# stdio2016/pfann

Measured on AMD Instinct MI355X. Metric: query segments/sec, 10 s @ SNR 0 queries vs 1M-segment db (exact flat IP top-100 + sequence match), higher is better.
Workload: dtype f32

## Files before the change

include/pfann_amd.h:

```cpp
#ifndef PFANN_AMD_H
#define PFANN_AMD_H

#include <stdint.h>

#ifdef __cplusplus
extern "C" {
#endif

#define PFANN_SEQSCORE_VERSION 20220625002LL


long long version(void);

int seq_score(void *index, const int64_t *song_pos, int n_songs, const float *query,
              int query_len, const int64_t *labels, int top_k, float *song_scores,
              int frame_shift_mul, float score_alpha);

const char *pfann_last_error(void);

typedef struct pfann_ctx pfann_ctx;

typedef struct pfann_config {
    int32_t segment_len;
    int32_t stft_n;
// ... 4 lines not shown
    int32_t log_mode;
    int32_t spec_norm_max;
    float   log_eps;
    int32_t d, h, u;
    int32_t fuller;
    int32_t activation;
    int32_t relu_after_bn;
    int32_t stride_t[8];
    int32_t stride_f[8];
    int32_t max_batch;
} pfann_config;

pfann_ctx *pfann_create(const pfann_config *cfg, int device);
void pfann_destroy(pfann_ctx *ctx);

int pfann_set_melbank(pfann_ctx *ctx, const float *fb_host, int n_freqs, int n_mels);

int pfann_load_weight(pfann_ctx *ctx, const char *name, const float *host, int64_t numel);
int pfann_weights_missing(pfann_ctx *ctx);

int pfann_melspec(pfann_ctx *ctx, const float *segs_dev, int64_t B, int64_t seg_stride,
                  int remove_mean, float *out_dev, void *stream);

int pfann_melspec_plan(pfann_ctx *ctx, int64_t B, int out[4]);

int pfann_encode(pfann_ctx *ctx, const float *mel_dev, int64_t B, float *emb_dev,
                 int normalize, void *stream);

int pfann_segment_embed(pfann_ctx *ctx, const float *wav_dev, int64_t B, int64_t seg_stride,
                        float *emb_dev, int normalize, void *stream);

int pfann_segment_embed_at(pfann_ctx *ctx, const float *wav_dev, const int64_t *starts_dev,
                           int64_t B, float *emb_dev, int normalize, void *stream);

int pfann_pcm16_to_mono(pfann_ctx *ctx, const int16_t *pcm_dev, int64_t n_frames, int n_ch,
                        float *wav_dev, void *stream);

int pfann_pcm16_files_to_mono(pfann_ctx *ctx, const void *const *host_pcm, const int64_t *n_samples, const int64_t *dst_off,
                              int n_files, int16_t *pcm_dev, int64_t total, float *wav_dev, void *stream);

typedef struct pfann_wav_info {
    int64_t n_frames;
    int64_t data_pos;
    int32_t n_ch;
    int32_t sample_rate;
    int32_t status;
    int32_t reserved;
// ... 213 lines not shown
```

pfann_amd/csrc/api.hip:

```cpp
#include <math.h>
#include <stdarg.h>
#include <stdlib.h>
#include <string.h>

#include <algorithm>
#include <cmath>
#include <map>
#include <mutex>

#include "kernels.h"
#include "search_plan.h"

namespace pfann { int launch_rows_to_half(const float *x, int64_t n, int d, void *xh, float *norm_max_dev, hipStream_t s); }

__global__ void noop_api_kernel() {}
static int launch_noop_api() {
    hipLaunchKernelGGL(noop_api_kernel, dim3(1), dim3(1), 0, 0);
    return hipGetLastError() == hipSuccess ? 0 : -1;
}

namespace pfann {

static thread_local char g_err[1024] = "";
void set_error(const char *fmt, ...) {
// ... 61 lines not shown
    int keep = 0;
    int64_t keep_first = 0;
    int64_t keep_B = 0;
    float *dbg[16] = {};
    bool dbg_has[16] = {};
    float *dbg_tmp = nullptr;
    int64_t dbg_cap = 0;
};

extern "C" int pfann_set_streams(pfann_ctx *c, int n);

static int build_plan(pfann_ctx *c) {
    const char *why = plan_sublayers(c->cfg, c->F, c->T, c->sub);
    if (why) { set_error("%s", why); return -1; }
    return 0;
}

static int upload(float **dst, const float *src, size_t n) {
    if (*dst == nullptr) PF_HIP(hipMalloc(dst, n * sizeof(float)));
    PF_HIP(hipMemcpy(*dst, src, n * sizeof(float), hipMemcpyHostToDevice));
    return 0;
}

__global__ void pfann_bench_region_marker() {}

extern "C" {

long long version(void) { return PFANN_SEQSCORE_VERSION; }

const char *pfann_last_error(void) { return g_err; }

pfann_ctx *pfann_create(const pfann_config *cfg, int device) {
    if (hipSetDevice(device) != hipSuccess) { set_error("hipSetDevice(%d) failed: no usable GPU", device); return nullptr; }
    pfann_ctx *c = new pfann_ctx();
    c->cfg = *cfg;
    c->device = device;
    if (c->cfg.max_batch <= 0) c->cfg.max_batch = 512;
    const int n_fft = cfg->stft_n;
    int log2n = 0;
    while ((1 << log2n) < n_fft) ++log2n;
    if ((1 << log2n) != n_fft || n_fft < 64 || n_fft > 4096) { set_error("stft_n must be a power of two in 64..4096"); delete c; return nullptr; }
    if (cfg->n_mels % 1 != 0 || cfg->n_mels <= 0) { set_error("bad n_mels"); delete c; return nullptr; }
    MelPlan &m = c->mel;
    memset(&m, 0, sizeof(m));
    m.seg_len = cfg->segment_len; m.n_fft = n_fft; m.hop = cfg->stft_hop; m.n_mels = cfg->n_mels;
    m.n_frames = 1 + cfg->segment_len / cfg->stft_hop;
    m.n_freqs = n_fft / 2 + 1; m.log2n = log2n;
    m.power = cfg->power; m.pad_reflect = cfg->pad_reflect; m.log_mode = cfg->log_mode;
    m.spec_norm_max = cfg->spec_norm_max; m.log_eps = cfg->log_eps;
    if (m.pad_reflect && n_fft / 2 >= cfg->segment_len) { set_error("reflect padding needs stft_n/2 < segment_len"); delete c; return nullptr; }
    std::vector<float> win(n_fft);
    std::vector<float2> tw(n_fft / 2);
    for (int n = 0; n < n_fft; ++n) win[n] = (float)(0.5 - 0.5 * cos(2.0 * M_PI * n / n_fft));
    for (int j = 0; j < n_fft / 2; ++j) {
        tw[j].x = (float)cos(-2.0 * M_PI * j / n_fft);
        tw[j].y = (float)sin(-2.0 * M_PI * j / n_fft);
    }
    if (hipMalloc(&m.window, n_fft * sizeof(float)) != hipSuccess ||
        hipMalloc(&m.twiddle, (n_fft / 2) * sizeof(float2)) != hipSuccess) { set_error("hipMalloc failed"); delete c; return nullptr; }
    (void)hipMemcpy(m.window, win.data(), n_fft * sizeof(float), hipMemcpyHostToDevice);
    (void)hipMemcpy(m.twiddle, tw.data(), (n_fft / 2) * sizeof(float2), hipMemcpyHostToDevice);
    c->F = cfg->n_mels;
    c->T = m.n_frames;
    if (build_plan(c)) { delete c; return nullptr; }
    c->n_expected = 8 * 8 + 4;
    for (int i = 0; i < 16; ++i) {
        const int64_t e = (int64_t)c->sub[i].co * c->sub[i].Fo * c->sub[i].To;
        c->buf_elems[i & 1] = std::max(c->buf_elems[i & 1], e);
    }
    c->fused = fused_supported(c->sub, 16) && getenv("PFANN_NO_FUSE") == nullptr;
    if (!c->fused && cfg->fuller && getenv("PFANN_NO_FUSE") == nullptr)
        fprintf(stderr, "pfann_amd: this model's layer shapes (an Fo*To that is not a power of two, or channel counts not "
// ... 17 lines not shown
        if (c->sub[i].w_hi) { (void)hipFree(c->sub[i].w_hi); (void)hipFree(c->sub[i].w_lo); }
        if (c->sub[i].w22) (void)hipFree(c->sub[i].w22);
        if (c->sub[i].bias) (void)hipFree(c->sub[i].bias);
        if (c->sub[i].ln_w) (void)hipFree(c->sub[i].ln_w);
        if (c->sub[i].ln_b) (void)hipFree(c->sub[i].ln_b);
        if (c->dbg[i]) (void)hipFree(c->dbg[i]);
    }
    float *ptrs[] = {c->g_w1, c->g_b1, c->g_w2, c->g_b2, c->buf[0], c->buf[1], c->part[0], c->part[1], c->splitk, c->stats, c->mel_buf, c->mel.window,
                     c->mel.fb_val, c->dbg_tmp};
    for (float *p : ptrs) if (p) (void)hipFree(p);
    if (c->mel.twiddle) (void)hipFree(c->mel.twiddle);
    if (c->mel.fb_ptr) (void)hipFree(c->mel.fb_ptr);
    if (c->mel.fb_idx) (void)hipFree(c->mel.fb_idx);
    if (c->scratch) (void)hipFree(c->scratch);
    delete c;
}

int pfann_set_melbank(pfann_ctx *c, const float *fb, int n_freqs, int n_mels) {
    if (n_freqs != c->mel.n_freqs || n_mels != c->mel.n_mels) {
        set_error("melbank shape [%d,%d] != [%d,%d]", n_freqs, n_mels, c->mel.n_freqs, c->mel.n_mels);
        return -3;
    }
    PF_HIP(hipSetDevice(c->device));
    std::vector<int> ptr(n_mels + 1, 0), idx;
    std::vector<float> val;
    int mx = 0;
    for (int m = 0; m < n_mels; ++m) {
        for (int k = 0; k < n_freqs; ++k) {
            const float v = fb[(size_t)k * n_mels + m];
            if (v != 0.0f) { idx.push_back(k); val.push_back(v); }
        }
        ptr[m + 1] = (int)idx.size();
        mx = std::max(mx, ptr[m + 1] - ptr[m]);
    }
    if (idx.empty()) { idx.push_back(0); val.push_back(0.f); }
    MelPlan &mp = c->mel;
    if (mp.fb_ptr) { (void)hipFree(mp.fb_ptr); (void)hipFree(mp.fb_idx); (void)hipFree(mp.fb_val); }
    PF_HIP(hipMalloc(&mp.fb_ptr, ptr.size() * sizeof(int)));
    PF_HIP(hipMalloc(&mp.fb_idx, idx.size() * sizeof(int)));
    PF_HIP(hipMalloc(&mp.fb_val, val.size() * sizeof(float)));
    PF_HIP(hipMemcpy(mp.fb_ptr, ptr.data(), ptr.size() * sizeof(int), hipMemcpyHostToDevice));
    PF_HIP(hipMemcpy(mp.fb_idx, idx.data(), idx.size() * sizeof(int), hipMemcpyHostToDevice));
    PF_HIP(hipMemcpy(mp.fb_val, val.data(), val.size() * sizeof(float), hipMemcpyHostToDevice));
    mp.max_nnz_row = mx;
    mp.fb_nnz = (int)idx.size();
    c->mel_ready = true;
    return 0;
}

int pfann_load_weight(pfann_ctx *c, const char *name, const float *host, int64_t numel) {
    PF_HIP(hipSetDevice(c->device));
    const pfann_config &g = c->cfg;
    int blk = -1;
    char mod[16] = "", kind[16] = "";
    if (sscanf(name, "f.convs.%d.%15[a-z0-9].%15s", &blk, mod, kind) == 3 && blk >= 0 && blk < 8) {
        const bool second = mod[strlen(mod) - 1] == '2';
        SubLayer &L = c->sub[2 * blk + (second ? 1 : 0)];
        const bool is_w = strcmp(kind, "weight") == 0;
        if (!is_w && strcmp(kind, "bias") != 0) { set_error("unknown tensor %s", name); return -2; }
        if (strncmp(mod, "conv", 4) == 0) {
            if (!is_w) {
                if (numel != L.co) { set_error("%s: numel %lld != %d", name, (long long)numel, L.co); return -3; }
                if (upload(&L.bias, host, numel)) return -1;
                if (blk == 0 && !second) { c->b1_host.assign(host, host + numel); c->gram_ready = false; }
            } else {
                const int ci = L.depthwise ? 1 : L.ci;
                if (numel != (int64_t)L.co * ci * 3) { set_error("%s: numel %lld != %lld", name, (long long)numel, (long long)L.co * ci * 3); return -3; }
                std::vector<float> w((size_t)numel);
// ... 56 lines not shown
        else if (!strcmp(name, "g.linear1.bias")) { dst = &c->g_b1; want = (int64_t)g.d * g.u; }
        else if (!strcmp(name, "g.linear2.weight")) { dst = &c->g_w2; want = (int64_t)g.d * g.u; }
        else if (!strcmp(name, "g.linear2.bias")) { dst = &c->g_b2; want = g.d; }
        else { set_error("unknown tensor %s", name); return -2; }
        if (numel != want) { set_error("%s: numel %lld != %lld", name, (long long)numel, (long long)want); return -3; }
        if (upload(dst, host, numel)) return -1;
    } else {
        set_error("unknown tensor %s", name);
        return -2;
    }
    c->loaded[name] = true;
    return 0;
}

int pfann_weights_missing(pfann_ctx *c) { return c->n_expected - (int)c->loaded.size(); }

int pfann_melspec(pfann_ctx *c, const float *segs, int64_t B, int64_t seg_stride, int remove_mean, float *out,
                  void *stream) {
    PF_HIP(hipSetDevice(c->device));
    if (!c->mel_ready) { set_error("pfann_melspec: mel filterbank not set"); return -5; }
    return launch_melspec(c->mel, segs, B, seg_stride, nullptr, remove_mean, out, (hipStream_t)stream);
}

int pfann_melspec_plan(pfann_ctx *c, int64_t B, int out[4]) {
    if (!c->mel_ready) { set_error("pfann_melspec_plan: mel filterbank not set"); return -5; }
    const MelLaunch ml = plan_melspec(c->mel, B);
    out[0] = ml.group_out; out[1] = ml.parts; out[2] = (int)ml.lds_bytes; out[3] = ml.radix8;
    return 0;
}

static int64_t keep_window(const pfann_ctx *c, int64_t B, int64_t *first) {
    const int64_t nb = std::min<int64_t>(B, 8);
    *first = std::max<int64_t>(0, std::min<int64_t>(c->keep_first, B - nb));
    return nb;
}

static int keep_tap(pfann_ctx *c, int idx, const float *act, int64_t B, hipStream_t s) {
    const SubLayer &L = c->sub[idx];
    const int64_t e = (int64_t)L.co * L.Fo * L.To;
    int64_t b0;
    const int64_t nb = keep_window(c, B, &b0);
    if (!c->dbg[idx]) PF_HIP(hipMalloc(&c->dbg[idx], 8 * e * sizeof(float)));
    PF_HIP(hipMemcpyAsync(c->dbg[idx], act + b0 * e, nb * e * sizeof(float), hipMemcpyDeviceToDevice, s));
    c->keep_B = nb;
    c->dbg_has[idx] = true;
    return 0;
}

static int ensure_workspace(pfann_ctx *c, bool need_mel) {
    const int64_t mb = c->cfg.max_batch;
// ... 1385 lines not shown
```

pfann_amd/csrc/kernels.h:

```cpp
#pragma once
#include "common.h"
#include "encoder_plan.h"

namespace pfann {

struct MelPlan {
    int seg_len, n_fft, hop, n_mels, n_frames, n_freqs, log2n;
    int power, pad_reflect, log_mode, spec_norm_max;
    float log_eps;
    float *window;
    float2 *twiddle;
    int *fb_ptr;
    int *fb_idx;
    float *fb_val;
    int max_nnz_row, fb_nnz;
};
struct MelLaunch {
    int group_out, parts, radix8;
    size_t lds_bytes;
};
MelLaunch plan_melspec(const MelPlan &mp, int64_t B);
int launch_melspec(const MelPlan &mp, const float *segs, int64_t B, int64_t seg_stride,
                   const int64_t *starts, int remove_mean, float *out, hipStream_t s);
int launch_resample_to_mono(const int16_t *pcm, int n_ch, const float *K, int old_r, int new_r, int width, const int64_t *plan,
                            int n_pieces, int64_t n_out, float *tmp, float *wav, float *scratch2, hipStream_t s);
int launch_pcm16_to_mono(const int16_t *pcm, int64_t n_frames, int n_ch, float *wav,
                         float *scratch2, hipStream_t s);

int launch_conv_first(const SubLayer &L, const float *x, float *y, int64_t B, hipStream_t s);
int launch_conv_gemm(const SubLayer &L, const float *x, float *y, int64_t B, hipStream_t s, int64_t Bcall = 0);
int launch_conv_depthwise(const SubLayer &L, const float *x, float *y, int64_t B, hipStream_t s);
int launch_ln_act(const SubLayer &L, float *xy, int64_t B, int activation, int relu_after_bn,
                  hipStream_t s);
int launch_myg(const float *x, const float *w1, const float *b1, const float *w2, const float *b2,
               int d, int u, int v, int64_t B, float *emb, int normalize, hipStream_t s);
int launch_cl_to_nchw(const float *x, float *y, int64_t B, int C, int HW, hipStream_t s);

bool fused_supported(const SubLayer *sub, int n);
int fused_out_slots(const SubLayer &L, int64_t B);
int launch_conv_first_stats(const SubLayer &L, const float *x, float *y, float *part, int64_t B, int act,
                            int after_bn, hipStream_t s);
int launch_conv_first_gram_stats(const SubLayer &L, const float *x, float *part, int64_t B, const float *gram14,
                                 hipStream_t s);
// ... 195 lines not shown
```

pfann_amd/csrc/mel.hip:

```cpp
#include <stdlib.h>

#include "kernels.h"

namespace pfann {

struct MelArgs {
    const float *segs; float *out;
    int64_t seg_stride;
    const int64_t *starts;
    int seg_len, n_fft, hop, n_mels, n_frames, log2n;
    int power, pad_reflect, log_mode, spec_norm_max, remove_mean;
    float log_eps;
    const float *window; const float2 *twiddle;
    const int *fb_ptr, *fb_idx; const float *fb_val;
    int fb_nnz;
    int parts;
    int group_out;
};

__device__ __forceinline__ unsigned bitrev(unsigned x, int bits) { return __brev(x) >> (32 - bits); }

__device__ __forceinline__ float2 cadd(float2 a, float2 b) { return make_float2(a.x + b.x, a.y + b.y); }
__device__ __forceinline__ float2 csub(float2 a, float2 b) { return make_float2(a.x - b.x, a.y - b.y); }
__device__ __forceinline__ float2 cmul(float2 a, float2 b) { return make_float2(a.x * b.x - a.y * b.y, a.x * b.y + a.y * b.x); }
__device__ __forceinline__ float2 mul_mi(float2 a) { return make_float2(a.y, -a.x); }

__device__ __forceinline__ void dft8(float2 (&a)[8]) {
    const float c = 0.70710678118654752440f;
    float2 u[8], v[8];
#pragma unroll
    for (int j = 0; j < 4; ++j) { u[j] = cadd(a[j], a[j + 4]); u[j + 4] = csub(a[j], a[j + 4]); }
    u[5] = make_float2(c * (u[5].x + u[5].y), c * (u[5].y - u[5].x));
    u[6] = mul_mi(u[6]);
    u[7] = make_float2(c * (u[7].y - u[7].x), -c * (u[7].x + u[7].y));
#pragma unroll
    for (int h = 0; h < 8; h += 4) {
        v[h] = cadd(u[h], u[h + 2]); v[h + 2] = csub(u[h], u[h + 2]);
        v[h + 1] = cadd(u[h + 1], u[h + 3]); v[h + 3] = mul_mi(csub(u[h + 1], u[h + 3]));
    }
    a[0] = cadd(v[0], v[1]); a[4] = csub(v[0], v[1]);
    a[2] = cadd(v[2], v[3]); a[6] = csub(v[2], v[3]);
    a[1] = cadd(v[4], v[5]); a[5] = csub(v[4], v[5]);
    a[3] = cadd(v[6], v[7]); a[7] = csub(v[6], v[7]);
}

__global__ __launch_bounds__(256) void melspec_kernel(MelArgs a) {
    extern __shared__ __attribute__((aligned(16))) float smem[];
    const int M = a.n_fft >> 1;
    const int log2m = a.log2n - 1;
    const int n_freqs = M + 1;
    float *tw_re = smem;
    float *tw_im = tw_re + M;
    const int WSZ = 2 * M > 1152 ? 2 * M : 1152;
    float *work = tw_im + M;
    float *pw = work + 4 * WSZ;
    float *tile = pw + 4 * (M + 4);
    const int tp = a.group_out ? a.group_out + 1 : a.n_frames + 1;
    float *red = tile + a.n_mels * tp;
    int *s_ptr = reinterpret_cast<int *>(red + 8);
    int *s_idx = s_ptr + a.n_mels + 1;
    float *s_val = reinterpret_cast<float *>(s_idx + a.fb_nnz);

    const int tid = threadIdx.x, lane = tid & 63, wave = tid >> 6;
    const int seg = a.parts > 1 ? (int)blockIdx.x / a.parts : (int)blockIdx.x, part = a.parts > 1 ? (int)blockIdx.x % a.parts : 0;
    const float *x = a.segs + (a.starts ? a.starts[seg] : (int64_t)seg * a.seg_stride);

    for (int j = tid; j < M; j += 256) { const float2 t = a.twiddle[j]; tw_re[j] = t.x; tw_im[j] = t.y; }
    for (int j = tid; j <= a.n_mels; j += 256) s_ptr[j] = a.fb_ptr[j];
    for (int j = tid; j < a.fb_nnz; j += 256) { s_idx[j] = a.fb_idx[j]; s_val[j] = a.fb_val[j]; }

    constexpr int SMAX = 32;
    const bool inreg = a.seg_len <= SMAX * 256;
    float xr[SMAX];
#pragma unroll
    for (int j = 0; j < SMAX; ++j) {
        const int i = tid + 256 * j;
        xr[j] = (inreg && i < a.seg_len) ? x[i] : 0.f;
    }
    float mean = 0.f;
    if (a.remove_mean) {
        float s = 0.f;
        if (inreg) {
#pragma unroll
            for (int j = 0; j < SMAX; ++j) if (tid + 256 * j < a.seg_len) s += xr[j];
        } else {
            for (int i = tid; i < a.seg_len; i += 256) s += x[i];
        }
        s = wave_sum(s);
        if (lane == 0) red[wave] = s;
        __syncthreads();
        mean = ((red[0] + red[1]) + (red[2] + red[3])) / (float)a.seg_len;
        __syncthreads();
// ... 16 lines not shown
                    if (tid + 256 * j < a.seg_len) { const float v = xr[j] - mean; s = fmaf(v, v, s); }
            } else {
                for (int i = tid; i < a.seg_len; i += 256) { const float v = x[i] - mean; s = fmaf(v, v, s); }
            }
            s = wave_sum(s);
        }
        if (lane == 0) red[4 + wave] = s;
        __syncthreads();
        const float t = a.spec_norm_max ? fmaxf(fmaxf(red[4], red[5]), fmaxf(red[6], red[7]))
                                        : sqrtf((red[4] + red[5]) + (red[6] + red[7]));
        denom = fmaxf(t, 1e-12f);
    }
    const float rden = 1.0f / denom;
    auto div_denom = [&](float v) {
        const float q = v * rden;
        return fmaf(fmaf(-q, denom, v), rden, q);
    };

    auto wave_sync = []() {
        __builtin_amdgcn_fence(__ATOMIC_RELEASE, "wavefront");
        __builtin_amdgcn_wave_barrier();
        __builtin_amdgcn_fence(__ATOMIC_ACQUIRE, "wavefront");
    };
    float *zre = work + wave * WSZ, *zim = zre + M, *pwr = pw + wave * (M + 4);
    const bool radix8 = a.n_fft == 1024;
    float win[8][2];
#pragma unroll
    for (int n1 = 0; n1 < 8; ++n1)
#pragma unroll
        for (int e = 0; e < 2; ++e) win[n1][e] = radix8 ? a.window[2 * (64 * n1 + lane) + e] : 0.f;
    float2 tw1[8], tw2[8];
#pragma unroll
    for (int j = 1; j < 8; ++j) {
        const int e1 = radix8 ? 2 * lane * j : 0, e2 = radix8 ? 16 * (lane & 7) * j : 0;
        tw1[j] = make_float2((e1 >= 512 ? -1.f : 1.f) * tw_re[e1 & 511], (e1 >= 512 ? -1.f : 1.f) * tw_im[e1 & 511]);
        tw2[j] = make_float2((e2 >= 512 ? -1.f : 1.f) * tw_re[e2 & 511], (e2 >= 512 ? -1.f : 1.f) * tw_im[e2 & 511]);
    }
    const int n_groups = (a.n_frames + 3) >> 2;
    const int g_lo = part * (n_groups / a.parts), g_hi = a.parts > 1 ? g_lo + n_groups / a.parts : n_groups;
    for (int g = g_lo; g < g_hi; ++g) {
        const int t = g * 4 + wave;
        const bool live = t < a.n_frames;
        if (radix8) {
            float2 *tb = reinterpret_cast<float2 *>(zre);
            float2 v[8];
#pragma unroll
            for (int n1 = 0; n1 < 8; ++n1) {
                const int m = 64 * n1 + lane;
                float w[2];
#pragma unroll
                for (int e = 0; e < 2; ++e) {
                    const int n = 2 * m + e;
                    int idx = t * a.hop - M + n;
                    float s = 0.f;
                    if (live) {
                        if (a.pad_reflect) {
                            if (idx < 0) idx = -idx;
                            if (idx > a.seg_len - 1) idx = 2 * (a.seg_len - 1) - idx;
                            s = div_denom(x[idx] - mean);
                        } else if (idx >= 0 && idx < a.seg_len) {
                            s = div_denom(x[idx] - mean);
                        }
                    }
                    w[e] = s * win[n1][e];
                }
                v[n1] = make_float2(w[0], w[1]);
            }
            const int hi = lane >> 3, lo = lane & 7;
            dft8(v);
#pragma unroll
            for (int k1 = 1; k1 < 8; ++k1) v[k1] = cmul(v[k1], tw1[k1]);
#pragma unroll
// ... 38 lines not shown
                    v[e] = s * a.window[n];
                }
                const unsigned r = bitrev((unsigned)m, log2m);
                zre[r] = v[0];
                zim[r] = v[1];
            }
            wave_sync();
            for (int s = 1; s <= log2m; ++s) {
                const int half = 1 << (s - 1);
                for (int bf = lane; bf < (M >> 1); bf += 64) {
                    const int grp = bf >> (s - 1), j = bf & (half - 1);
                    const int i0 = (grp << s) + j, i1 = i0 + half;
                    const int k = (j << (log2m - s)) << 1;
                    const float wr = tw_re[k], wi = tw_im[k];
                    const float xr = zre[i1], xi = zim[i1];
                    const float tr = wr * xr - wi * xi, ti = wr * xi + wi * xr;
                    const float ur = zre[i0], ui = zim[i0];
                    zre[i0] = ur + tr; zim[i0] = ui + ti;
                    zre[i1] = ur - tr; zim[i1] = ui - ti;
                }
                wave_sync();
            }
        }
        for (int k = lane; k <= M; k += 64) {
            const int k0 = k & (M - 1), k1 = (M - k) & (M - 1);
            const float ar = zre[k0], ai = zim[k0], br = zre[k1], bi = -zim[k1];
            const float er = 0.5f * (ar + br), ei = 0.5f * (ai + bi);
            const float dr = 0.5f * (ar - br), di = 0.5f * (ai - bi);
            const float orr = di, oi = -dr;
            float wr, wi;
            if (k < M) { wr = tw_re[k]; wi = tw_im[k]; } else { wr = -1.f; wi = 0.f; }
            const float xr = er + (wr * orr - wi * oi), xi = ei + (wr * oi + wi * orr);
            const float p2 = xr * xr + xi * xi;
            pwr[k] = a.power == 2 ? p2 : sqrtf(p2);
        }
        wave_sync();
        if (live) {
            for (int m = lane; m < a.n_mels; m += 64) {
                float acc = 0.f;
                const int e1 = s_ptr[m + 1];
                int e = s_ptr[m];
                for (; e + 3 < e1; e += 4) {
                    const float v0 = s_val[e], v1 = s_val[e + 1], v2 = s_val[e + 2], v3 = s_val[e + 3];
                    const float p0 = pwr[s_idx[e]], p1 = pwr[s_idx[e + 1]], p2 = pwr[s_idx[e + 2]], p3 = pwr[s_idx[e + 3]];
                    acc = fmaf(v0, p0, acc); acc = fmaf(v1, p1, acc); acc = fmaf(v2, p2, acc); acc = fmaf(v3, p3, acc);
                }
                for (; e < e1; ++e) acc = fmaf(s_val[e], pwr[s_idx[e]], acc);
                acc += a.log_eps;
                if (a.log_mode == 1) acc = logf(acc);
                else if (a.log_mode == 2) acc = log10f(acc);
                if (a.group_out) tile[m * tp + (t % a.group_out)] = acc;
                else tile[m * tp + t] = acc;
            }
        }
        wave_sync();
        if (a.group_out && ((4 * g + 4) % a.group_out == 0)) {
            __syncthreads();
            const int q4 = a.group_out >> 2;
            float *og = a.out + (int64_t)seg * a.n_mels * a.n_frames + (4 * g + 4 - a.group_out);
            for (int i = tid; i < a.n_mels * q4; i += 256) {
                const int m = i / q4, c = i - m * q4;
                const float *tr = tile + m * tp + 4 * c;
                *reinterpret_cast<float4 *>(og + (int64_t)m * a.n_frames + 4 * c) = make_float4(tr[0], tr[1], tr[2], tr[3]);
            }
            __syncthreads();
        }
    }
    if (a.group_out) return;
    __syncthreads();
    float sub = 0.f;
    if (a.spec_norm_max) {
        float mx = -INFINITY;
        for (int i = tid; i < a.n_mels * a.n_frames; i += 256)
            mx = fmaxf(mx, tile[(i / a.n_frames) * (a.n_frames + 1) + (i % a.n_frames)]);
        mx = wave_max(mx);
        if (lane == 0) red[wave] = mx;
        __syncthreads();
        sub = fmaxf(fmaxf(red[0], red[1]), fmaxf(red[2], red[3]));
    }
    float *o = a.out + (int64_t)seg * a.n_mels * a.n_frames;
    if (256 % a.n_frames == 0) {
        const int tf = tid % a.n_frames, mstep = 256 / a.n_frames;
        int m = tid / a.n_frames;
        for (int i = tid; i < a.n_mels * a.n_frames; i += 256, m += mstep) o[i] = tile[m * (a.n_frames + 1) + tf] - sub;
    } else {
        for (int i = tid; i < a.n_mels * a.n_frames; i += 256)
            o[i] = tile[(i / a.n_frames) * (a.n_frames + 1) + (i % a.n_frames)] - sub;
    }
}

MelLaunch plan_melspec(const MelPlan &mp, int64_t B) {
    MelLaunch ml;
    const int M = mp.n_fft / 2;
    const int WSZ = 2 * M > 1152 ? 2 * M : 1152;
    auto lds_for = [&](int gf) {
        return sizeof(float) * (size_t)(2 * M + 4 * WSZ + 4 * (M + 4) + mp.n_mels * (gf ? gf + 1 : mp.n_frames + 1) + 8 +
                                        mp.n_mels + 1 + 2 * (size_t)mp.fb_nnz);
    };
    ml.group_out = 0;
    if (!mp.spec_norm_max) {
        for (int gf : {16, 8, 4})
            if (mp.n_frames % gf == 0 && (ml.group_out == 0 ? (3 * lds_for(gf) <= 160 * 1024 || gf == 4) : false)) ml.group_out = gf;
    }
    if (getenv("PFANN_MEL_GROUP")) ml.group_out = atoi(getenv("PFANN_MEL_GROUP"));
    ml.parts = 1;
    if (ml.group_out && B <= 192 && mp.n_frames % ml.group_out == 0 && (mp.n_frames / ml.group_out) * ml.group_out == mp.n_frames &&
        ml.group_out % 4 == 0 && mp.n_frames % 4 == 0)
        ml.parts = mp.n_frames / ml.group_out;
    ml.lds_bytes = lds_for(ml.group_out);
    ml.radix8 = mp.n_fft == 1024 ? 1 : 0;
    return ml;
}

int launch_melspec(const MelPlan &mp, const float *segs, int64_t B, int64_t seg_stride, const int64_t *starts,
                   int remove_mean, float *out, hipStream_t s) {
    if (B <= 0) return 0;
    MelArgs a;
    a.segs = segs; a.out = out; a.seg_stride = seg_stride; a.starts = starts;
    a.seg_len = mp.seg_len; a.n_fft = mp.n_fft; a.hop = mp.hop; a.n_mels = mp.n_mels;
    a.n_frames = mp.n_frames; a.log2n = mp.log2n;
    a.power = mp.power; a.pad_reflect = mp.pad_reflect; a.log_mode = mp.log_mode;
    a.spec_norm_max = mp.spec_norm_max; a.remove_mean = remove_mean; a.log_eps = mp.log_eps;
    a.window = mp.window; a.twiddle = mp.twiddle;
    a.fb_ptr = mp.fb_ptr; a.fb_idx = mp.fb_idx; a.fb_val = mp.fb_val; a.fb_nnz = mp.fb_nnz;
    const MelLaunch ml = plan_melspec(mp, B);
    a.group_out = ml.group_out;
    a.parts = ml.parts;
    const size_t lds = ml.lds_bytes;
    if (lds > 160 * 1024) { set_error("melspec: LDS need %zu B > 160 KiB", lds); return -1; }
    if (ensure_dyn_lds((const void *)melspec_kernel, 160 * 1024)) return -1;
    ProfScope ps("melspec", s);
    PF_LAUNCH(melspec_kernel, dim3((unsigned)(B * a.parts)), dim3(256), lds, s, a);
    PF_HIP(hipGetLastError());
    return 0;
}

__global__ void stereo_power_kernel(const int16_t *__restrict__ pcm, int64_t n, double *pw) {
    double p1 = 0, p2 = 0;
    for (int64_t i = (int64_t)blockIdx.x * blockDim.x + threadIdx.x; i < n; i += (int64_t)gridDim.x * blockDim.x) {
        const float l = (float)pcm[2 * i] * (1.0f / 32768.0f), r = (float)pcm[2 * i + 1] * (1.0f / 32768.0f);
        p1 += (double)((l - r) * (l - r));
        p2 += (double)((l + r) * (l + r));
    }
    p1 = wave_sum_d(p1); p2 = wave_sum_d(p2);
    if ((threadIdx.x & 63) == 0) { atomicAdd(&pw[0], p1); atomicAdd(&pw[1], p2); }
}
__global__ void pcm_to_mono_kernel(const int16_t *__restrict__ pcm, int64_t n, int n_ch, const double *pw,
                                   float *__restrict__ wav) {
    const int64_t i = (int64_t)blockIdx.x * blockDim.x + threadIdx.x;
    if (i >= n) return;
    if (n_ch == 1) { wav[i] = (float)pcm[i] * (1.0f / 32768.0f); return; }
    float acc = 0.f;
    const bool flip = n_ch == 2 && (float)(pw[0] / (double)n) > (float)(pw[1] / (double)n) * 1000.0f;
    for (int c = 0; c < n_ch; ++c) {
        float v = (float)pcm[i * n_ch + c] * (1.0f / 32768.0f);
// ... 119 lines not shown
```

pfann_amd/engine.py:

```python
import ctypes

import numpy as np
import torch

from . import lib as _l
from .config import config_from_params
from .synth import model_dims


def _mel_to_hz_tensor(m, scale):
    if scale == "htk":
        return 700.0 * (10.0 ** (m / 2595.0) - 1.0)
    import math
    logstep = math.log(6.4) / 27.0
    return torch.where(m >= 15.0, 1000.0 * torch.exp(logstep * (m - 15.0)), (200.0 / 3) * m)


def _hz_to_mel(f, scale):
    import math
    if scale == "htk":
        return 2595.0 * math.log10(1.0 + f / 700.0)
    if f >= 1000.0:
        return 15.0 + math.log(f / 1000.0) / (math.log(6.4) / 27.0)
    return f / (200.0 / 3)
# ... 17 lines not shown
    lib = _l.load()
    size = 1 << 16
    while True:
        buf = ctypes.create_string_buffer(size)
        rc = lib.pfann_encode_plan(ctypes.byref(cfg), int(B), int(plan_batch), int(precision), int(fused), int(taps), int(streams),
                                   buf, len(buf))
        if rc != -2 or size >= 1 << 24:
            break
        size *= 4
    _l.check(rc, "pfann_encode_plan")
    lines = buf.value.decode().splitlines()
    assert lines[-1].startswith("flags "), lines[-1]
    launches, chunk_info = [], []
    for ln in lines[:-1]:
        if ln.startswith("chunk "):
            chunk_info.append({k: int(v) for k, v in (kv.split("=") for kv in ln.split(" ")[2:])})
            continue
        name, rest = ln.rsplit(" grid=", 1)
        d = {k: int(v) for k, v in (kv.split("=") for kv in ("grid=" + rest).split(" "))}
        launches.append(dict(d, name=name, chunk=len(chunk_info) - 1))
    flags = {k: int(v) for k, v in (kv.split("=") for kv in lines[-1].split(" ")[1:])}
    flags["chunk_info"] = chunk_info
    return launches, flags


class Engine:
    def __init__(self, params, device=0, max_batch=512, encoder_only=False):
        _l.require_gpu()
        self.encoder_only = encoder_only
        self.lib = _l.load()
        self.params = params
        self.device = torch.device("cuda", device if isinstance(device, int) else (device.index or 0))
        self.cfg = config_from_params(params, max_batch)
        self.d, self.h, self.u, self.F, self.T = model_dims(params)
        self.seg_len = self.cfg.segment_len
        from . import prewarm
        self.handle = prewarm.take_engine(self.cfg, self.device.index) if not encoder_only else None
        self.weights_loaded = self.handle is not None
        if self.handle is None:
            self.handle = self.lib.pfann_create(ctypes.byref(self.cfg), self.device.index)
        self._resample_tables = {}
        self.before_front_end = None
        if not self.handle:
            raise _l.PfannError("pfann_create failed: " + _l.last_error())
        n_frames = 1 + self.seg_len // self.cfg.stft_hop
        if n_frames != self.T:
# ... 26 lines not shown
            x = torch.as_tensor(np.asarray(x, dtype=np.float32))
        return x.to(self.device, torch.float32).contiguous()

    def _need_front_end(self, what):
        if self.encoder_only:
            raise _l.PfannError("%s: this Engine was built encoder-only (FpNetwork without a full config); build it from "
                                "the whole configs/*.json dict" % what)

    def melspec(self, segs):
        self._need_front_end("melspec")
        if self.before_front_end is not None:
            self.before_front_end()
        x = self._prep(segs)
        lead = x.shape[:-1]
        x2 = x.reshape(-1, self.seg_len)
        out = torch.empty((x2.shape[0], self.F, self.T), device=self.device, dtype=torch.float32)
        if x2.shape[0]:
            _l.check(self.lib.pfann_melspec(self.handle, x2.data_ptr(), x2.shape[0], self.seg_len, 0,
                                            out.data_ptr(), self._stream()), "pfann_melspec")
        return out.reshape(*lead, self.F, self.T)

    def melspec_plan(self, B):
        self._need_front_end("melspec_plan")
        out = (ctypes.c_int * 4)()
        _l.check(self.lib.pfann_melspec_plan(self.handle, int(B), out), "pfann_melspec_plan")
        return {"group_out": out[0], "parts": out[1], "lds_bytes": out[2], "radix8": bool(out[3]),
                "in_register": self.seg_len <= 8192}

    def encode(self, mel, norm=True):
        x = self._prep(mel)
        assert x.dim() == 3 and x.shape[1] == self.F and x.shape[2] == self.T, x.shape
        out = torch.empty((x.shape[0], self.d), device=self.device, dtype=torch.float32)
        if x.shape[0]:
            _l.check(self.lib.pfann_encode(self.handle, x.data_ptr(), x.shape[0], out.data_ptr(),
                                           1 if norm else 0, self._stream()), "pfann_encode")
        return out

    def embed_wav(self, wav, hop, n_seg=None, norm=True):
        self._need_front_end("embed_wav")
        if self.before_front_end is not None:
            self.before_front_end()
        w = self._prep(wav).reshape(-1)
        if w.shape[0] < self.seg_len:
            w = torch.nn.functional.pad(w, (0, self.seg_len - w.shape[0]))
        if n_seg is None:
            n_seg = (w.shape[0] - self.seg_len) // hop + 1
        assert (n_seg - 1) * hop + self.seg_len <= w.shape[0]
        out = torch.empty((n_seg, self.d), device=self.device, dtype=torch.float32)
        if n_seg:
            _l.check(self.lib.pfann_segment_embed(self.handle, w.data_ptr(), n_seg, hop, out.data_ptr(),
# ... 91 lines not shown
```

pfann_amd/lib.py:

```python
import ctypes
import os
from ctypes import (POINTER, Structure, c_char_p, c_double, c_float, c_int, c_int16, c_int32, c_int64,
                    c_longlong, c_void_p)

HERE = os.path.dirname(os.path.abspath(__file__))
LIB_PATH = os.path.join(HERE, "libpfann_amd.so")


class PfannError(RuntimeError):
    pass


class Config(Structure):
    _fields_ = [("segment_len", c_int32), ("stft_n", c_int32), ("stft_hop", c_int32), ("n_mels", c_int32),
                ("power", c_int32), ("pad_reflect", c_int32), ("log_mode", c_int32),
                ("spec_norm_max", c_int32), ("log_eps", c_float),
                ("d", c_int32), ("h", c_int32), ("u", c_int32), ("fuller", c_int32),
                ("activation", c_int32), ("relu_after_bn", c_int32),
                ("stride_t", c_int32 * 8), ("stride_f", c_int32 * 8), ("max_batch", c_int32)]


class MatchResult(Structure):
    _fields_ = [("song", c_int32), ("offset", c_int32), ("shift", c_int32), ("n_cand", c_int32),
                ("score", c_double)]


class WavInfo(Structure):
    _fields_ = [("n_frames", c_int64), ("data_pos", c_int64), ("n_ch", c_int32), ("sample_rate", c_int32),
                ("status", c_int32), ("reserved", c_int32)]


SYMBOLS = {
    "version": (c_longlong, []),
    "seq_score": (c_int, [c_void_p, POINTER(c_int64), c_int, POINTER(c_float), c_int, POINTER(c_int64),
                          c_int, POINTER(c_float), c_int, c_float]),
    "pfann_last_error": (c_char_p, []),
    "pfann_create": (c_void_p, [POINTER(Config), c_int]),
    "pfann_destroy": (None, [c_void_p]),
    "pfann_set_melbank": (c_int, [c_void_p, c_void_p, c_int, c_int]),
    "pfann_load_weight": (c_int, [c_void_p, c_char_p, c_void_p, c_int64]),
    "pfann_weights_missing": (c_int, [c_void_p]),
    "pfann_melspec": (c_int, [c_void_p, c_void_p, c_int64, c_int64, c_int, c_void_p, c_void_p]),
    "pfann_melspec_plan": (c_int, [c_void_p, c_int64, POINTER(c_int)]),
    "pfann_encode": (c_int, [c_void_p, c_void_p, c_int64, c_void_p, c_int, c_void_p]),
    "pfann_segment_embed": (c_int, [c_void_p, c_void_p, c_int64, c_int64, c_void_p, c_int, c_void_p]),
    "pfann_segment_embed_at": (c_int, [c_void_p, c_void_p, c_void_p, c_int64, c_void_p, c_int, c_void_p]),
    "pfann_pcm16_to_mono": (c_int, [c_void_p, c_void_p, c_int64, c_int, c_void_p, c_void_p]),
    "pfann_pcm16_files_to_mono": (c_int, [c_void_p, POINTER(c_void_p), POINTER(c_int64), POINTER(c_int64), c_int, c_void_p, c_int64,
                                          c_void_p, c_void_p]),
    "pfann_wav_probe": (c_int, [POINTER(c_char_p), c_int, c_int, POINTER(WavInfo)]),
    "pfann_wav_read": (c_int, [POINTER(c_char_p), c_int, c_int, POINTER(WavInfo), POINTER(c_int64), c_void_p, c_int64]),
    "pfann_resample_to_mono": (c_int, [c_void_p, c_void_p, c_int, c_void_p, c_int, c_int, c_int, c_void_p, c_int, c_int64,
                                       c_void_p, c_void_p, c_void_p]),
    "pfann_debug_activation": (c_int64, [c_void_p, c_int, c_int64, c_void_p, c_int64]),
    "pfann_debug_keep": (None, [c_void_p, c_int]),
    "pfann_debug_keep_at": (c_int, [c_void_p, c_int, c_int64]),
    "pfann_encode_plan": (c_int, [POINTER(Config), c_int64, c_int64, c_int, c_int, c_int, c_int, c_char_p, c_int]),
    "pfann_set_fused_layernorm": (c_int, [c_void_p, c_int]),
    "pfann_set_encoder_precision": (c_int, [c_void_p, c_int]),
    "pfann_prewarm": (c_int, [c_int]),
    "pfann_set_plan_batch": (c_int64, [c_void_p, c_int64]),
    "pfann_set_streams": (c_int, [c_void_p, c_int]),
    "pfann_db_create": (c_void_p, [c_int, c_int]),
    "pfann_db_destroy": (None, [c_void_p]),
    "pfann_db_set_prefilter": (c_int, [c_void_p, c_int]),
    "pfann_db_set_storage": (c_int, [c_void_p, c_int]),
# ... 135 lines not shown
```

Before: 214,200.

## Slim melspec kernel LDS footprint with lean radix-8 path and contiguous mel bank

Templates the melspec kernel into radix-8, radix-2 and legacy V1 variants. The radix-8 variant no longer stages twiddles in LDS and reuses the FFT work buffer for the power spectrum. When every mel filter row covers contiguous frequency bins, it also packs the start index into the row pointer and drops the index array. This shrinks LDS per block, and a launch-bounds hint of 5 waves is meant to allow more resident blocks, at the cost of more global/cache reads for twiddles and window values and extra code complexity.

```diff
diff --git a/include/pfann_amd.h b/include/pfann_amd.h
--- a/include/pfann_amd.h
+++ b/include/pfann_amd.h
@@ -50,7 +50,9 @@
 int pfann_melspec(pfann_ctx *ctx, const float *segs_dev, int64_t B, int64_t seg_stride,
                   int remove_mean, float *out_dev, void *stream);
 
-int pfann_melspec_plan(pfann_ctx *ctx, int64_t B, int out[4]);
+int pfann_melspec_plan(pfann_ctx *ctx, int64_t B, int out[5]);
+
+int pfann_melspec_plan_host(const pfann_config *cfg, const float *fb, int n_freqs, int n_mels, int64_t B, int out[5]);
 
 int pfann_encode(pfann_ctx *ctx, const float *mel_dev, int64_t B, float *emb_dev,
                  int normalize, void *stream);
diff --git a/pfann_amd/csrc/api.hip b/pfann_amd/csrc/api.hip
--- a/pfann_amd/csrc/api.hip
+++ b/pfann_amd/csrc/api.hip
@@ -107,6 +107,39 @@
     return 0;
 }
 
+static const char *mel_plan_from_config(const pfann_config &cfg, MelPlan &m) {
+    const int n_fft = cfg.stft_n;
+    int log2n = 0;
+    while ((1 << log2n) < n_fft) ++log2n;
+    if ((1 << log2n) != n_fft || n_fft < 64 || n_fft > 4096) return "stft_n must be a power of two in 64..4096";
+    if (cfg.n_mels <= 0) return "bad n_mels";
+    memset(&m, 0, sizeof(m));
+    m.seg_len = cfg.segment_len; m.n_fft = n_fft; m.hop = cfg.stft_hop; m.n_mels = cfg.n_mels;
+    m.n_frames = 1 + cfg.segment_len / cfg.stft_hop;
+    m.n_freqs = n_fft / 2 + 1; m.log2n = log2n;
+    m.power = cfg.power; m.pad_reflect = cfg.pad_reflect; m.log_mode = cfg.log_mode;
+    m.spec_norm_max = cfg.spec_norm_max; m.log_eps = cfg.log_eps;
+    return nullptr;
+}
+
+static void mel_bank_csr(const float *fb, int n_freqs, int n_mels, std::vector<int> &ptr, std::vector<int> &idx,
+                         std::vector<float> &val, MelPlan &mp) {
+    ptr.assign(n_mels + 1, 0);
+    int mx = 0;
+    for (int m = 0; m < n_mels; ++m) {
+        for (int k = 0; k < n_freqs; ++k) {
+            const float v = fb[(size_t)k * n_mels + m];
+            if (v != 0.0f) { idx.push_back(k); val.push_back(v); }
+        }
+        ptr[m + 1] = (int)idx.size();
+        mx = std::max(mx, ptr[m + 1] - ptr[m]);
+    }
+    if (idx.empty()) { idx.push_back(0); val.push_back(0.f); }
+    mp.max_nnz_row = mx;
+    mp.fb_nnz = (int)idx.size();
+    mp.fb_contiguous = mel_bank_contiguous(ptr.data(), idx.data(), n_mels) ? 1 : 0;
+}
+
 __global__ void pfann_bench_region_marker() {}
 
 extern "C" {
@@ -121,18 +154,9 @@
     c->cfg = *cfg;
     c->device = device;
     if (c->cfg.max_batch <= 0) c->cfg.max_batch = 512;
-    const int n_fft = cfg->stft_n;
-    int log2n = 0;
-    while ((1 << log2n) < n_fft) ++log2n;
-    if ((1 << log2n) != n_fft || n_fft < 64 || n_fft > 4096) { set_error("stft_n must be a power of two in 64..4096"); delete c; return nullptr; }
-    if (cfg->n_mels % 1 != 0 || cfg->n_mels <= 0) { set_error("bad n_mels"); delete c; return nullptr; }
     MelPlan &m = c->mel;
-    memset(&m, 0, sizeof(m));
-    m.seg_len = cfg->segment_len; m.n_fft = n_fft; m.hop = cfg->stft_hop; m.n_mels = cfg->n_mels;
-    m.n_frames = 1 + cfg->segment_len / cfg->stft_hop;
-    m.n_freqs = n_fft / 2 + 1; m.log2n = log2n;
-    m.power = cfg->power; m.pad_reflect = cfg->pad_reflect; m.log_mode = cfg->log_mode;
-    m.spec_norm_max = cfg->spec_norm_max; m.log_eps = cfg->log_eps;
+    if (const char *why = mel_plan_from_config(*cfg, m)) { set_error("%s", why); delete c; return nullptr; }
+    const int n_fft = m.n_fft;
     if (m.pad_reflect && n_fft / 2 >= cfg->segment_len) { set_error("reflect padding needs stft_n/2 < segment_len"); delete c; return nullptr; }
     std::vector<float> win(n_fft);
     std::vector<float2> tw(n_fft / 2);
@@ -196,19 +220,10 @@
         return -3;
     }
     PF_HIP(hipSetDevice(c->device));
-    std::vector<int> ptr(n_mels + 1, 0), idx;
+    MelPlan &mp = c->mel;
+    std::vector<int> ptr, idx;
     std::vector<float> val;
-    int mx = 0;
-    for (int m = 0; m < n_mels; ++m) {
-        for (int k = 0; k < n_freqs; ++k) {
-            const float v = fb[(size_t)k * n_mels + m];
-            if (v != 0.0f) { idx.push_back(k); val.push_back(v); }
-        }
-        ptr[m + 1] = (int)idx.size();
-        mx = std::max(mx, ptr[m + 1] - ptr[m]);
-    }
-    if (idx.empty()) { idx.push_back(0); val.push_back(0.f); }
-    MelPlan &mp = c->mel;
+    mel_bank_csr(fb, n_freqs, n_mels, ptr, idx, val, mp);
     if (mp.fb_ptr) { (void)hipFree(mp.fb_ptr); (void)hipFree(mp.fb_idx); (void)hipFree(mp.fb_val); }
     PF_HIP(hipMalloc(&mp.fb_ptr, ptr.size() * sizeof(int)));
     PF_HIP(hipMalloc(&mp.fb_idx, idx.size() * sizeof(int)));
@@ -216,8 +231,6 @@
     PF_HIP(hipMemcpy(mp.fb_ptr, ptr.data(), ptr.size() * sizeof(int), hipMemcpyHostToDevice));
     PF_HIP(hipMemcpy(mp.fb_idx, idx.data(), idx.size() * sizeof(int), hipMemcpyHostToDevice));
     PF_HIP(hipMemcpy(mp.fb_val, val.data(), val.size() * sizeof(float), hipMemcpyHostToDevice));
-    mp.max_nnz_row = mx;
-    mp.fb_nnz = (int)idx.size();
     c->mel_ready = true;
     return 0;
 }
@@ -320,10 +333,25 @@
     return launch_melspec(c->mel, segs, B, seg_stride, nullptr, remove_mean, out, (hipStream_t)stream);
 }
 
-int pfann_melspec_plan(pfann_ctx *c, int64_t B, int out[4]) {
+int pfann_melspec_plan(pfann_ctx *c, int64_t B, int out[5]) {
     if (!c->mel_ready) { set_error("pfann_melspec_plan: mel filterbank not set"); return -5; }
     const MelLaunch ml = plan_melspec(c->mel, B);
-    out[0] = ml.group_out; out[1] = ml.parts; out[2] = (int)ml.lds_bytes; out[3] = ml.radix8;
+    out[0] = ml.group_out; out[1] = ml.parts; out[2] = (int)ml.lds_bytes; out[3] = ml.radix8; out[4] = ml.contiguous_bank;
+    return 0;
+}
+
+int pfann_melspec_plan_host(const pfann_config *cfg, const float *fb, int n_freqs, int n_mels, int64_t B, int out[5]) {
+    MelPlan mp;
+    if (const char *why = mel_plan_from_config(*cfg, mp)) { set_error("%s", why); return -3; }
+    if (n_freqs != mp.n_freqs || n_mels != mp.n_mels) {
+        set_error("melbank shape [%d,%d] != [%d,%d]", n_freqs, n_mels, mp.n_freqs, mp.n_mels);
+        return -3;
+    }
+    std::vector<int> ptr, idx;
+    std::vector<float> val;
+    mel_bank_csr(fb, n_freqs, n_mels, ptr, idx, val, mp);
+    const MelLaunch ml = plan_melspec(mp, B);
+    out[0] = ml.group_out; out[1] = ml.parts; out[2] = (int)ml.lds_bytes; out[3] = ml.radix8; out[4] = ml.contiguous_bank;
     return 0;
 }
 
diff --git a/pfann_amd/csrc/kernels.h b/pfann_amd/csrc/kernels.h
--- a/pfann_amd/csrc/kernels.h
+++ b/pfann_amd/csrc/kernels.h
@@ -14,11 +14,13 @@
     int *fb_idx;
     float *fb_val;
     int max_nnz_row, fb_nnz;
+    int fb_contiguous;
 };
 struct MelLaunch {
-    int group_out, parts, radix8;
+    int group_out, parts, radix8, contiguous_bank, v1;
     size_t lds_bytes;
 };
+bool mel_bank_contiguous(const int *ptr, const int *idx, int n_mels);
 MelLaunch plan_melspec(const MelPlan &mp, int64_t B);
 int launch_melspec(const MelPlan &mp, const float *segs, int64_t B, int64_t seg_stride,
                    const int64_t *starts, int remove_mean, float *out, hipStream_t s);
diff --git a/pfann_amd/csrc/mel.hip b/pfann_amd/csrc/mel.hip
--- a/pfann_amd/csrc/mel.hip
+++ b/pfann_amd/csrc/mel.hip
@@ -14,6 +14,7 @@
     const float *window; const float2 *twiddle;
     const int *fb_ptr, *fb_idx; const float *fb_val;
     int fb_nnz;
+    int fb_contig;
     int parts;
     int group_out;
 };
@@ -44,30 +45,42 @@
     a[3] = cadd(v[6], v[7]); a[7] = csub(v[6], v[7]);
 }
 
-__global__ __launch_bounds__(256) void melspec_kernel(MelArgs a) {
+template <bool V1, bool R8>
+__device__ __forceinline__ void melspec_body(const MelArgs &a) {
     extern __shared__ __attribute__((aligned(16))) float smem[];
     const int M = a.n_fft >> 1;
     const int log2m = a.log2n - 1;
-    const int n_freqs = M + 1;
+    const bool radix8 = V1 ? a.n_fft == 1024 : R8;
+    const bool lean = !V1 && radix8;
+    const bool contig = !V1 && a.fb_contig;
     float *tw_re = smem;
     float *tw_im = tw_re + M;
     const int WSZ = 2 * M > 1152 ? 2 * M : 1152;
-    float *work = tw_im + M;
+    float *work = lean ? smem : tw_im + M;
     float *pw = work + 4 * WSZ;
-    float *tile = pw + 4 * (M + 4);
+    float *tile = lean ? pw : pw + 4 * (M + 4);
     const int tp = a.group_out ? a.group_out + 1 : a.n_frames + 1;
     float *red = tile + a.n_mels * tp;
     int *s_ptr = reinterpret_cast<int *>(red + 8);
     int *s_idx = s_ptr + a.n_mels + 1;
-    float *s_val = reinterpret_cast<float *>(s_idx + a.fb_nnz);
+    float *s_val = reinterpret_cast<float *>(contig ? s_idx : s_idx + a.fb_nnz);
 
     const int tid = threadIdx.x, lane = tid & 63, wave = tid >> 6;
     const int seg = a.parts > 1 ? (int)blockIdx.x / a.parts : (int)blockIdx.x, part = a.parts > 1 ? (int)blockIdx.x % a.parts : 0;
     const float *x = a.segs + (a.starts ? a.starts[seg] : (int64_t)seg * a.seg_stride);
 
-    for (int j = tid; j < M; j += 256) { const float2 t = a.twiddle[j]; tw_re[j] = t.x; tw_im[j] = t.y; }
-    for (int j = tid; j <= a.n_mels; j += 256) s_ptr[j] = a.fb_ptr[j];
-    for (int j = tid; j < a.fb_nnz; j += 256) { s_idx[j] = a.fb_idx[j]; s_val[j] = a.fb_val[j]; }
+    if (!lean)
+        for (int j = tid; j < M; j += 256) { const float2 t = a.twiddle[j]; tw_re[j] = t.x; tw_im[j] = t.y; }
+    if (contig) {
+        for (int j = tid; j <= a.n_mels; j += 256) {
+            const int p = a.fb_ptr[j];
+            s_ptr[j] = (int)((unsigned)p | ((unsigned)(p < a.fb_nnz ? a.fb_idx[p] : 0) << 20));
+        }
+        for (int j = tid; j < a.fb_nnz; j += 256) s_val[j] = a.fb_val[j];
+    } else {
+        for (int j = tid; j <= a.n_mels; j += 256) s_ptr[j] = a.fb_ptr[j];
+        for (int j = tid; j < a.fb_nnz; j += 256) { s_idx[j] = a.fb_idx[j]; s_val[j] = a.fb_val[j]; }
+    }
 
     constexpr int SMAX = 32;
     const bool inreg = a.seg_len <= SMAX * 256;
@@ -130,19 +143,20 @@
         __builtin_amdgcn_wave_barrier();
         __builtin_amdgcn_fence(__ATOMIC_ACQUIRE, "wavefront");
     };
-    float *zre = work + wave * WSZ, *zim = zre + M, *pwr = pw + wave * (M + 4);
-    const bool radix8 = a.n_fft == 1024;
+    float *zre = work + wave * WSZ, *zim = zre + M, *pwr = lean ? zre : pw + wave * (M + 4);
     float win[8][2];
 #pragma unroll
     for (int n1 = 0; n1 < 8; ++n1)
 #pragma unroll
-        for (int e = 0; e < 2; ++e) win[n1][e] = radix8 ? a.window[2 * (64 * n1 + lane) + e] : 0.f;
+        for (int e = 0; e < 2; ++e) win[n1][e] = V1 && radix8 ? a.window[2 * (64 * n1 + lane) + e] : 0.f;
     float2 tw1[8], tw2[8];
 #pragma unroll
     for (int j = 1; j < 8; ++j) {
         const int e1 = radix8 ? 2 * lane * j : 0, e2 = radix8 ? 16 * (lane & 7) * j : 0;
-        tw1[j] = make_float2((e1 >= 512 ? -1.f : 1.f) * tw_re[e1 & 511], (e1 >= 512 ? -1.f : 1.f) * tw_im[e1 & 511]);
-        tw2[j] = make_float2((e2 >= 512 ? -1.f : 1.f) * tw_re[e2 & 511], (e2 >= 512 ? -1.f : 1.f) * tw_im[e2 & 511]);
+        const float2 t1 = V1 ? make_float2(tw_re[e1 & 511], tw_im[e1 & 511]) : a.twiddle[e1 & 511];
+        const float2 t2 = V1 ? make_float2(tw_re[e2 & 511], tw_im[e2 & 511]) : a.twiddle[e2 & 511];
+        tw1[j] = make_float2((e1 >= 512 ? -1.f : 1.f) * t1.x, (e1 >= 512 ? -1.f : 1.f) * t1.y);
+        tw2[j] = make_float2((e2 >= 512 ? -1.f : 1.f) * t2.x, (e2 >= 512 ? -1.f : 1.f) * t2.y);
     }
     const int n_groups = (a.n_frames + 3) >> 2;
     const int g_lo = part * (n_groups / a.parts), g_hi = a.parts > 1 ? g_lo + n_groups / a.parts : n_groups;
@@ -156,6 +170,7 @@
             for (int n1 = 0; n1 < 8; ++n1) {
                 const int m = 64 * n1 + lane;
                 float w[2];
+                if (!V1) { const float2 wn = *reinterpret_cast<const float2 *>(a.window + 2 * m); win[n1][0] = wn.x; win[n1][1] = wn.y; }
 #pragma unroll
                 for (int e = 0; e < 2; ++e) {
                     const int n = 2 * m + e;
@@ -240,30 +255,65 @@
                 wave_sync();
             }
         }
-        for (int k = lane; k <= M; k += 64) {
-            const int k0 = k & (M - 1), k1 = (M - k) & (M - 1);
+        auto split_power = [&](int k0, int k1, float wr, float wi) {
             const float ar = zre[k0], ai = zim[k0], br = zre[k1], bi = -zim[k1];
             const float er = 0.5f * (ar + br), ei = 0.5f * (ai + bi);
             const float dr = 0.5f * (ar - br), di = 0.5f * (ai - bi);
             const float orr = di, oi = -dr;
-            float wr, wi;
-            if (k < M) { wr = tw_re[k]; wi = tw_im[k]; } else { wr = -1.f; wi = 0.f; }
             const float xr = er + (wr * orr - wi * oi), xi = ei + (wr * oi + wi * orr);
-            const float p2 = xr * xr + xi * xi;
-            pwr[k] = a.power == 2 ? p2 : sqrtf(p2);
+            return xr * xr + xi * xi;
+        };
+        if (lean) {
+            float pv[9];
+            int kr = 64 - lane;
+            asm volatile("" : "+v"(kr));
+#pragma unroll
+            for (int j = 0; j < 8; ++j) {
+                const float2 w = a.twiddle[lane + 64 * j];
+                pv[j] = split_power(lane + 64 * j, j == 0 && lane == 0 ? 0 : kr + 64 * (7 - j), w.x, w.y);
+            }
+            pv[8] = split_power(0, 0, -1.f, 0.f);
+            if (a.power != 2) {
+#pragma unroll
+                for (int j = 0; j < 9; ++j) pv[j] = sqrtf(pv[j]);
+            }
+            wave_sync();
+#pragma unroll
+            for (int j = 0; j < 8; ++j) pwr[lane + 64 * j] = pv[j];
+            if (lane == 0) pwr[512] = pv[8];
+        } else {
+            for (int k = lane; k <= M; k += 64) {
+                float wr, wi;
+                if (k < M) { wr = tw_re[k]; wi = tw_im[k]; } else { wr = -1.f; wi = 0.f; }
+                const float p2 = split_power(k & (M - 1), (M - k) & (M - 1), wr, wi);
+                pwr[k] = a.power == 2 ? p2 : sqrtf(p2);
+            }
         }
         wave_sync();
         if (live) {
             for (int m = lane; m < a.n_mels; m += 64) {
                 float acc = 0.f;
-                const int e1 = s_ptr[m + 1];
-                int e = s_ptr[m];
-                for (; e + 3 < e1; e += 4) {
-                    const float v0 = s_val[e], v1 = s_val[e + 1], v2 = s_val[e + 2], v3 = s_val[e + 3];
-                    const float p0 = pwr[s_idx[e]], p1 = pwr[s_idx[e + 1]], p2 = pwr[s_idx[e + 2]], p3 = pwr[s_idx[e + 3]];
-                    acc = fmaf(v0, p0, acc); acc = fmaf(v1, p1, acc); acc = fmaf(v2, p2, acc); acc = fmaf(v3, p3, acc);
+                if (contig) {
+                    const int w0 = s_ptr[m];
+                    const int e1 = s_ptr[m + 1] & 0xfffff;
+                    int e = w0 & 0xfffff;
+                    const float *pr = pwr + ((int)((unsigned)w0 >> 20) - e);
+                    for (; e + 3 < e1; e += 4) {
+                        const float v0 = s_val[e], v1 = s_val[e + 1], v2 = s_val[e + 2], v3 = s_val[e + 3];
+                        const float p0 = pr[e], p1 = pr[e + 1], p2 = pr[e + 2], p3 = pr[e + 3];
+                        acc = fmaf(v0, p0, acc); acc = fmaf(v1, p1, acc); acc = fmaf(v2, p2, acc); acc = fmaf(v3, p3, acc);
+                    }
+                    for (; e < e1; ++e) acc = fmaf(s_val[e], pr[e], acc);
+                } else {
+                    const int e1 = s_ptr[m + 1];
+                    int e = s_ptr[m];
+                    for (; e + 3 < e1; e += 4) {
+                        const float v0 = s_val[e], v1 = s_val[e + 1], v2 = s_val[e + 2], v3 = s_val[e + 3];
+                        const float p0 = pwr[s_idx[e]], p1 = pwr[s_idx[e + 1]], p2 = pwr[s_idx[e + 2]], p3 = pwr[s_idx[e + 3]];
+                        acc = fmaf(v0, p0, acc); acc = fmaf(v1, p1, acc); acc = fmaf(v2, p2, acc); acc = fmaf(v3, p3, acc);
+                    }
+                    for (; e < e1; ++e) acc = fmaf(s_val[e], pwr[s_idx[e]], acc);
                 }
-                for (; e < e1; ++e) acc = fmaf(s_val[e], pwr[s_idx[e]], acc);
                 acc += a.log_eps;
                 if (a.log_mode == 1) acc = logf(acc);
                 else if (a.log_mode == 2) acc = log10f(acc);
@@ -275,7 +325,9 @@
         if (a.group_out && ((4 * g + 4) % a.group_out == 0)) {
             __syncthreads();
             const int q4 = a.group_out >> 2;
-            float *og = a.out + (int64_t)seg * a.n_mels * a.n_frames + (4 * g + 4 - a.group_out);
+            int sg = seg;
+            if (!V1) { sg = __builtin_amdgcn_readfirstlane(sg); asm volatile("" : "+s"(sg)); }
+            float *og = a.out + (int64_t)sg * a.n_mels * a.n_frames + (4 * g + 4 - a.group_out);
             for (int i = tid; i < a.n_mels * q4; i += 256) {
                 const int m = i / q4, c = i - m * q4;
                 const float *tr = tile + m * tp + 4 * c;
@@ -307,26 +359,49 @@
     }
 }
 
+__global__ __launch_bounds__(256, 5) void melspec_kernel(MelArgs a) { melspec_body<false, true>(a); }
+__global__ __launch_bounds__(256) void melspec_radix2_kernel(MelArgs a) { melspec_body<false, false>(a); }
+__global__ __launch_bounds__(256) void melspec_v1_kernel(MelArgs a) { melspec_body<true, false>(a); }
+
+static bool mel_v1() {
+    static const bool v1 = getenv("PFANN_MEL_V1") != nullptr && atoi(getenv("PFANN_MEL_V1")) != 0;
+    return v1;
+}
+
+bool mel_bank_contiguous(const int *ptr, const int *idx, int n_mels) {
+    for (int m = 0; m < n_mels; ++m)
+        for (int e = ptr[m] + 1; e < ptr[m + 1]; ++e)
+            if (idx[e] != idx[e - 1] + 1) return false;
+    return true;
+}
+
 MelLaunch plan_melspec(const MelPlan &mp, int64_t B) {
     MelLaunch ml;
     const int M = mp.n_fft / 2;
     const int WSZ = 2 * M > 1152 ? 2 * M : 1152;
-    auto lds_for = [&](int gf) {
-        return sizeof(float) * (size_t)(2 * M + 4 * WSZ + 4 * (M + 4) + mp.n_mels * (gf ? gf + 1 : mp.n_frames + 1) + 8 +
-                                        mp.n_mels + 1 + 2 * (size_t)mp.fb_nnz);
+    ml.radix8 = mp.n_fft == 1024 ? 1 : 0;
+    ml.v1 = mel_v1() ? 1 : 0;
+    ml.contiguous_bank = !ml.v1 && mp.fb_contiguous ? 1 : 0;
+    const bool lean = !ml.v1 && ml.radix8;
+    auto tile_floats = [&](int gf) { return (size_t)mp.n_mels * (gf ? gf + 1 : mp.n_frames + 1); };
+    auto v1_lds_bytes = [&](int gf) {
+        return sizeof(float) * (size_t)(2 * M + 4 * WSZ + 4 * (M + 4) + tile_floats(gf) + 8 + mp.n_mels + 1 + 2 * (size_t)mp.fb_nnz);
+    };
+    auto lds_bytes = [&](int gf) {
+        return sizeof(float) * (size_t)((lean ? 0 : 2 * M + 4 * (M + 4)) + 4 * WSZ + tile_floats(gf) + 8 + mp.n_mels + 1 +
+                                        (ml.contiguous_bank ? 1 : 2) * (size_t)mp.fb_nnz);
     };
     ml.group_out = 0;
     if (!mp.spec_norm_max) {
         for (int gf : {16, 8, 4})
-            if (mp.n_frames % gf == 0 && (ml.group_out == 0 ? (3 * lds_for(gf) <= 160 * 1024 || gf == 4) : false)) ml.group_out = gf;
+            if (mp.n_frames % gf == 0 && (ml.group_out == 0 ? (3 * v1_lds_bytes(gf) <= 160 * 1024 || gf == 4) : false)) ml.group_out = gf;
     }
     if (getenv("PFANN_MEL_GROUP")) ml.group_out = atoi(getenv("PFANN_MEL_GROUP"));
     ml.parts = 1;
     if (ml.group_out && B <= 192 && mp.n_frames % ml.group_out == 0 && (mp.n_frames / ml.group_out) * ml.group_out == mp.n_frames &&
         ml.group_out % 4 == 0 && mp.n_frames % 4 == 0)
         ml.parts = mp.n_frames / ml.group_out;
-    ml.lds_bytes = lds_for(ml.group_out);
-    ml.radix8 = mp.n_fft == 1024 ? 1 : 0;
+    ml.lds_bytes = ml.v1 ? v1_lds_bytes(ml.group_out) : lds_bytes(ml.group_out);
     return ml;
 }
 
@@ -342,13 +417,15 @@
     a.window = mp.window; a.twiddle = mp.twiddle;
     a.fb_ptr = mp.fb_ptr; a.fb_idx = mp.fb_idx; a.fb_val = mp.fb_val; a.fb_nnz = mp.fb_nnz;
     const MelLaunch ml = plan_melspec(mp, B);
+    a.fb_contig = ml.contiguous_bank;
     a.group_out = ml.group_out;
     a.parts = ml.parts;
     const size_t lds = ml.lds_bytes;
     if (lds > 160 * 1024) { set_error("melspec: LDS need %zu B > 160 KiB", lds); return -1; }
-    if (ensure_dyn_lds((const void *)melspec_kernel, 160 * 1024)) return -1;
-    ProfScope ps("melspec", s);
-    PF_LAUNCH(melspec_kernel, dim3((unsigned)(B * a.parts)), dim3(256), lds, s, a);
+    void (*const kernel)(MelArgs) = ml.v1 ? melspec_v1_kernel : ml.radix8 ? melspec_kernel : melspec_radix2_kernel;
+    if (ensure_dyn_lds((const void *)kernel, 160 * 1024)) return -1;
+    ProfScope ps("melspec", s, 4.0 * (double)B * ((double)mp.seg_len + (double)mp.n_mels * mp.n_frames));
+    PF_LAUNCH(kernel, dim3((unsigned)(B * a.parts)), dim3(256), lds, s, a);
     PF_HIP(hipGetLastError());
     return 0;
 }
diff --git a/pfann_amd/engine.py b/pfann_amd/engine.py
--- a/pfann_amd/engine.py
+++ b/pfann_amd/engine.py
@@ -63,6 +63,19 @@
     flags = {k: int(v) for k, v in (kv.split("=") for kv in lines[-1].split(" ")[1:])}
     flags["chunk_info"] = chunk_info
     return launches, flags
+
+
+def _melspec_plan_dict(out, seg_len):
+    return {"group_out": out[0], "parts": out[1], "lds_bytes": out[2], "radix8": bool(out[3]),
+            "in_register": seg_len <= 8192, "contiguous_bank": bool(out[4])}
+
+
+def melspec_plan_host(cfg, bank, B):
+    fb = np.ascontiguousarray(bank.numpy() if isinstance(bank, torch.Tensor) else bank, dtype=np.float32)
+    out = (ctypes.c_int * 5)()
+    _l.check(_l.load().pfann_melspec_plan_host(ctypes.byref(cfg), fb.ctypes.data, fb.shape[0], fb.shape[1], int(B), out),
+             "pfann_melspec_plan_host")
+    return _melspec_plan_dict(out, cfg.segment_len)
 
 
 class Engine:
@@ -135,10 +148,9 @@
 
     def melspec_plan(self, B):
         self._need_front_end("melspec_plan")
-        out = (ctypes.c_int * 4)()
+        out = (ctypes.c_int * 5)()
         _l.check(self.lib.pfann_melspec_plan(self.handle, int(B), out), "pfann_melspec_plan")
-        return {"group_out": out[0], "parts": out[1], "lds_bytes": out[2], "radix8": bool(out[3]),
-                "in_register": self.seg_len <= 8192}
+        return _melspec_plan_dict(out, self.seg_len)
 
     def encode(self, mel, norm=True):
         x = self._prep(mel)
diff --git a/pfann_amd/lib.py b/pfann_amd/lib.py
--- a/pfann_amd/lib.py
+++ b/pfann_amd/lib.py
@@ -42,6 +42,7 @@
     "pfann_weights_missing": (c_int, [c_void_p]),
     "pfann_melspec": (c_int, [c_void_p, c_void_p, c_int64, c_int64, c_int, c_void_p, c_void_p]),
     "pfann_melspec_plan": (c_int, [c_void_p, c_int64, POINTER(c_int)]),
+    "pfann_melspec_plan_host": (c_int, [POINTER(Config), c_void_p, c_int, c_int, c_int64, POINTER(c_int)]),
     "pfann_encode": (c_int, [c_void_p, c_void_p, c_int64, c_void_p, c_int, c_void_p]),
     "pfann_segment_embed": (c_int, [c_void_p, c_void_p, c_int64, c_int64, c_void_p, c_int, c_void_p]),
     "pfann_segment_embed_at": (c_int, [c_void_p, c_void_p, c_void_p, c_int64, c_void_p, c_int, c_void_p]),
```

Result: no change. 215,200, median of 6 (+0.5%).
